# REEVALUATE/knowledge_enhanced_multimodal_retrieval

Measured on AMD Instinct MI355X. Metric: gallery images+texts encoded/sec (ViT-L/14; synthetic texts per SURVEY 8(d): end-of-text uniform in positions 8..76, mean 43.8 of 77 positions computed -- value_every_text_77_positions is the rate when every text fills the context) and 43k x Q sim+top-10 ms, higher is better.
Workload: dtype bf16; 1 GPU; CLIP ViT-L/14 zero-shot: 43k-gallery encode (1 image + query + target text per item, 224x224 / 77 tokens) + T2I top-10, BASELINE configs[1]; architecture=ViT-L/14, residual_stream=fp24, batch_per_gpu=255, text_group=1501, gallery=43000, parallelism=dp1 (gallery sharded), rccl_ranks=1

## Files before the change

knowledge_enhanced_multimodal_retrieval_amd/csrc/attention.hip:

```cpp
#include "common.h"

namespace kemr {

#ifndef KEMR_ATTN_PRIO
#define KEMR_ATTN_PRIO 0
#endif
__device__ __forceinline__ void attn_prio(int mfma_phase) {
    if constexpr (KEMR_ATTN_PRIO == 1) { if (mfma_phase) __builtin_amdgcn_s_setprio(1); else __builtin_amdgcn_s_setprio(0); }
    if constexpr (KEMR_ATTN_PRIO == 2) { if (mfma_phase) __builtin_amdgcn_s_setprio(0); else __builtin_amdgcn_s_setprio(1); }
}

template <bool NT>
__device__ __forceinline__ bf16x8 load_q8(const bf16_t* p) {
    if constexpr (NT) return __builtin_nontemporal_load((const bf16x8*)p);
    else return *(const bf16x8*)p;
}

template <int NT32, bool CAUSAL, int TC, int NW = 4, bool STAMP = false, int NTLOAD = 1, bool SKIPTAIL = false>
__global__ __launch_bounds__(NW * 64, 2) void attention_kernel(const bf16_t* __restrict__ qkv, bf16_t* __restrict__ out,
                                                           int T_rt, int width, int xbatch, const int* __restrict__ row_start) {
    constexpr int TP = NT32 * 32;
    constexpr int NT16 = NT32 * 2;
    constexpr int NTH = NW * 64;
    constexpr int NCH = (TP * 8 + NTH - 1) / NTH;
    constexpr float LOG2E = 1.4426950408889634f;
    extern __shared__ __attribute__((aligned(16))) char smem[];
    char* sK = smem;
    char* sV = smem + TP * 128;

    int h, b;
    if (!attn_item(xbatch, h, b)) return;
    int T_ = TC > 0 ? TC : T_rt;
    size_t row0 = (size_t)b * T_;
    if (TC == 0 && row_start) {
        const int r0 = row_start[b];
        T_ = row_start[b + 1] - r0;
        row0 = r0;
    }
    const int T = T_;
    const int tid = threadIdx.x, lane = tid & 63;
    const int wid = __builtin_amdgcn_readfirstlane(tid >> 6);
    const int ld = 3 * width;
    const bf16_t* base = qkv + row0 * ld + h * 64;
    const int lrow = lane & 15, lq = lane >> 4;
    const int nqt = SKIPTAIL ? T >> 4 : (T + 15) >> 4;

    unsigned long long st_t[8] = {0, 0, 0, 0, 0, 0, 0, 0}, st_prev = 0;
    auto stamp = [&](int k) {
        if constexpr (STAMP) {
            __builtin_amdgcn_sched_barrier(0);
            unsigned long long now;
            asm volatile("s_memtime %0\n\ts_waitcnt lgkmcnt(0)" : "=s"(now) :: "memory");
            __builtin_amdgcn_sched_barrier(0);
            st_t[k] += now - st_prev;
            st_prev = now;
        }
    };
    if constexpr (STAMP) { asm volatile("s_memtime %0\n\ts_waitcnt lgkmcnt(0)" : "=s"(st_prev) :: "memory"); __builtin_amdgcn_sched_barrier(0); }
    bf16x8 qn[2];
    {
        const int q0 = wid * 16 + lrow;
        const int qc = q0 < T ? q0 : T - 1;
#pragma unroll
        for (int kk = 0; kk < 2; ++kk) qn[kk] = load_q8<(NTLOAD >= 2)>(base + (size_t)qc * ld + kk * 32 + lq * 8);
    }
    {
        uint4 kv[NCH], vv[NCH];
#pragma unroll
        for (int i = 0; i < NCH; ++i) {
            const int idx = tid + i * NTH;
            const int row = idx >> 3, c = idx & 7;
            const int rc = row < T ? row : T - 1;
            if constexpr (NTLOAD >= 1) {
                typedef unsigned u32x4_ __attribute__((ext_vector_type(4)));
                const u32x4_ a_ = __builtin_nontemporal_load((const u32x4_*)(base + (size_t)rc * ld + width + c * 8));
                const u32x4_ b_ = __builtin_nontemporal_load((const u32x4_*)(base + (size_t)rc * ld + 2 * width + c * 8));
                kv[i] = make_uint4(a_.x, a_.y, a_.z, a_.w);
                vv[i] = make_uint4(b_.x, b_.y, b_.z, b_.w);
            } else {
                kv[i] = *(const uint4*)(base + (size_t)rc * ld + width + c * 8);
                vv[i] = *(const uint4*)(base + (size_t)rc * ld + 2 * width + c * 8);
            }
        }
#pragma unroll
        for (int i = 0; i < NCH; ++i) {
            const int idx = tid + i * NTH;
            const int row = idx >> 3, c = idx & 7;
            if (idx < TP * 8) {
                const unsigned keep = row < T ? 0xffffffffu : 0u;
                uint4 a = kv[i], b2 = vv[i];
                a.x &= keep; a.y &= keep; a.z &= keep; a.w &= keep;
                b2.x &= keep; b2.y &= keep; b2.z &= keep; b2.w &= keep;
                *(uint4*)(sK + row * 128 + ((c ^ ((row >> 1) & 7)) << 4)) = a;
                *(uint4*)(sV + row * 128 + ((c ^ (((row >> 1) & 3) << 1)) << 4)) = b2;
            }
        }
    }
    __syncthreads();
    stamp(0);

    for (int qt = wid; qt < nqt; qt += NW) {
        const int q = qt * 16 + lrow;
        bf16x8 qf[2] = {qn[0], qn[1]};
        if (qt + NW < nqt) {
            const int q2 = q + NW * 16;
            const int qc = q2 < T ? q2 : T - 1;
#pragma unroll
            for (int kk = 0; kk < 2; ++kk) qn[kk] = load_q8<(NTLOAD >= 2)>(base + (size_t)qc * ld + kk * 32 + lq * 8);
        }

        constexpr int G = (NT16 % 3 == 0) ? 3 : 2;
        constexpr int NG = NT16 / G;
        f32x4 s[NT16];
        bf16x8 kfr[2][G][2];
        auto load_group = [&](int g, bf16x8 (&dst)[G][2]) {
#pragma unroll
            for (int j = 0; j < G; ++j)
#pragma unroll
                for (int kk = 0; kk < 2; ++kk)
                    dst[j][kk] = *(const bf16x8*)(sK + ((g * G + j) * 16 + lrow) * 128 + (((kk * 4 + lq) ^ (lrow >> 1)) << 4));
        };
        load_group(0, kfr[0]);
        attn_prio(1);
#pragma unroll
        for (int g = 0; g < NG; ++g) {
            if (g + 1 < NG && (g + 1) * G * 16 < T) load_group(g + 1, kfr[(g + 1) & 1]);
            __builtin_amdgcn_sched_barrier(0);
#pragma unroll
            for (int j = 0; j < G; ++j) {
                const int t = g * G + j;
                s[t] = f32x4{0.f, 0.f, 0.f, 0.f};
                if (t * 16 < T && (!CAUSAL || t <= qt)) {
                    s[t] = __builtin_amdgcn_mfma_f32_16x16x32_bf16(kfr[g & 1][j][0], qf[0], s[t], 0, 0, 0);
                    s[t] = __builtin_amdgcn_mfma_f32_16x16x32_bf16(kfr[g & 1][j][1], qf[1], s[t], 0, 0, 0);
                }
            }
            __builtin_amdgcn_sched_barrier(0);
        }
        attn_prio(0);
        stamp(1);
        float mx = -INFINITY;
#pragma unroll
        for (int t = 0; t < NT16; ++t) {
            const bool partial = (t + 1) * 16 > T || CAUSAL;
#pragma unroll
            for (int r = 0; r < 4; ++r) {
                if (partial) {
                    const int key = t * 16 + lq * 4 + r;
                    const bool ok = key < T && (!CAUSAL || key <= q);
                    s[t][r] = ok ? s[t][r] : -INFINITY;
                }
                mx = fmaxf(mx, s[t][r]);
            }
        }
        mx = fmaxf(mx, __shfl_xor(mx, 16));
        mx = fmaxf(mx, __shfl_xor(mx, 32));
        const float mxl = mx * LOG2E;
        stamp(2);
        f32x2_t sum2 = {0.f, 0.f};
        const f32x2_t l2 = {LOG2E, LOG2E}, nm = {-mxl, -mxl};
        auto exp_tile = [&](int t) {
            f32x2_t a = f32x2_t{s[t][0], s[t][1]} * l2 + nm, c = f32x2_t{s[t][2], s[t][3]} * l2 + nm;
            a.x = __builtin_amdgcn_exp2f(a.x); a.y = __builtin_amdgcn_exp2f(a.y);
            c.x = __builtin_amdgcn_exp2f(c.x); c.y = __builtin_amdgcn_exp2f(c.y);
            s[t][0] = a.x; s[t][1] = a.y; s[t][2] = c.x; s[t][3] = c.y;
            sum2 += a;
            sum2 += c;
        };
#pragma unroll
        for (int t = 0; t < NT16; ++t) exp_tile(t);

        stamp(3);
        f32x4 o[4];
#pragma unroll
        for (int dt = 0; dt < 4; ++dt) o[dt] = f32x4{0.f, 0.f, 0.f, 0.f};
        bf16x8 vfr[2][4];
        auto load_v = [&](int u, bf16x8 (&dst)[4]) {
            const int ra = u * 32 + lq * 4 + (lrow >> 2);
            const int rb = ra + 16;
#pragma unroll
            for (int dt = 0; dt < 4; ++dt) {
                const int c = dt * 2 + ((lrow & 3) >> 1);
                const bf16x4 va = lds_read_tr16(sV + ra * 128 + ((c ^ (((ra >> 1) & 3) << 1)) << 4) + (lrow & 1) * 8);
                const bf16x4 vb = lds_read_tr16(sV + rb * 128 + ((c ^ (((rb >> 1) & 3) << 1)) << 4) + (lrow & 1) * 8);
                dst[dt][0] = va[0]; dst[dt][1] = va[1]; dst[dt][2] = va[2]; dst[dt][3] = va[3];
                dst[dt][4] = vb[0]; dst[dt][5] = vb[1]; dst[dt][6] = vb[2]; dst[dt][7] = vb[3];
            }
        };
        load_v(0, vfr[0]);
        attn_prio(1);
        auto live = [&](int u) { return u < NT32 && u * 32 < T && !(CAUSAL && u * 32 > qt * 16 + 15); };
#pragma unroll
        for (int u = 0; u < NT32; ++u) {
            if (!live(u)) continue;
            if (u + 1 < NT32 && (u + 1) * 32 < T) load_v(u + 1, vfr[(u + 1) & 1]);
            __builtin_amdgcn_sched_barrier(0);
            union { bf16x8 v; uint32_t w[4]; } pf;
            pf.w[0] = pack_bf16x2(s[2 * u][0], s[2 * u][1]);
            pf.w[1] = pack_bf16x2(s[2 * u][2], s[2 * u][3]);
            pf.w[2] = pack_bf16x2(s[2 * u + 1][0], s[2 * u + 1][1]);
            pf.w[3] = pack_bf16x2(s[2 * u + 1][2], s[2 * u + 1][3]);
#pragma unroll
            for (int dt = 0; dt < 4; ++dt)
                o[dt] = __builtin_amdgcn_mfma_f32_16x16x32_bf16(vfr[u & 1][dt], pf.v, o[dt], 0, 0, 0);
            __builtin_amdgcn_sched_barrier(0);
        }
        attn_prio(0);
        stamp(4);
        float sum = sum2.x + sum2.y;
        sum += __shfl_xor(sum, 16);
        sum += __shfl_xor(sum, 32);
        if (q < T) {
            const float inv = 1.0f / sum;
            bf16_t* dst = out + (row0 + q) * width + h * 64 + lq * 4;
#pragma unroll
            for (int dt = 0; dt < 4; ++dt) {
                uint2 pk;
                pk.x = pack_bf16x2(o[dt][0] * inv, o[dt][1] * inv);
                pk.y = pack_bf16x2(o[dt][2] * inv, o[dt][3] * inv);
                *(uint2*)(dst + dt * 16) = pk;
            }
        }
        stamp(5);
    }
    if constexpr (STAMP) {
        unsigned long long* dst = (unsigned long long*)(out + (size_t)xbatch * T * width) + (((size_t)b * (width >> 6) + h) * NW + wid) * 8;
        if (lane == 0) {
#pragma unroll
            for (int k = 0; k < 6; ++k) dst[k] += st_t[k];
            dst[6] += 1;
        }
    }
}

int g_attn_v = 0;

int g_attn_xcd = 1;
int g_attn_waves = 0;

#ifdef KEMR_AB_VARIANTS
int launch_attention_ab(int v, int waves, const bf16_t* qkv, bf16_t* out, int batch, int width, int xbatch, hipStream_t stream);
#endif

template <int NT32>
static int launch_nt(const bf16_t* qkv, bf16_t* out, int batch, int t, int width, int causal, hipStream_t stream, const int* row_start = nullptr) {
    constexpr int smem = NT32 * 32 * 128 * 2;
    const dim3 grid(width / 64, batch);
    ProfScope prof(PROF_ATTENTION, stream);
    void (*kern)(const bf16_t*, bf16_t*, int, int, int, const int*);
    const int xbatch = g_attn_xcd ? batch : 0;
    const dim3 xgrid(width / 64, xbatch ? (batch + 7) / 8 * 8 : batch);
    int threads = 256;
    if (causal) {
        if (NT32 == 3 && t == 77 && !row_start) { kern = attention_kernel<NT32, true, NT32 == 3 ? 77 : 0, NT32 == 3 ? 5 : 4>; threads = 320; }
        else kern = attention_kernel<NT32, true, 0>;
    } else if (NT32 == 9 && t == 257) {
#ifdef KEMR_AB_VARIANTS
        if (g_attn_v != 0) return launch_attention_ab(g_attn_v, g_attn_waves, qkv, out, batch, width, xbatch, stream);
        if (g_attn_waves == 6) { kern = attention_kernel<NT32, false, NT32 == 9 ? 257 : 0, NT32 == 9 ? 6 : 4>; threads = 384; }
        else if (g_attn_waves == 7) kern = attention_kernel<NT32, false, NT32 == 9 ? 257 : 0, 4, false, NT32 == 9 ? 0 : 1>;
        else if (g_attn_waves == 8) kern = attention_kernel<NT32, false, NT32 == 9 ? 257 : 0, 4, false, 1, NT32 == 9>;
        else if (g_attn_waves == 5) kern = attention_kernel<NT32, false, NT32 == 9 ? 257 : 0, 4, false, NT32 == 9 ? 2 : 1>;
        else if (g_attn_waves == 2 && xbatch) kern = attention_kernel<NT32, false, NT32 == 9 ? 257 : 0, 4, NT32 == 9>;
        else
#else
        if (g_attn_v != 0 || g_attn_waves != 0)
            KEMR_FAIL(KEMR_ERR_INVALID, "attention: attn_v = %d / attn_waves = %d select A/B kernels this library was built without (build.py --ab-variants)", g_attn_v, g_attn_waves);
#endif
        kern = attention_kernel<NT32, false, NT32 == 9 ? 257 : 0>;
    } else {
        kern = attention_kernel<NT32, false, 0>;
    }
    KEMR_CHECK_HIP(hipFuncSetAttribute((const void*)kern, hipFuncAttributeMaxDynamicSharedMemorySize, smem));
    hipLaunchKernelGGL(kern, xgrid, dim3(threads), smem, stream, qkv, out, t, width, xbatch, row_start);
    KEMR_CHECK_LAUNCH("attention_kernel");
    return KEMR_OK;
}

int launch_attention(const bf16_t* qkv, bf16_t* out, int batch, int t, int width, int causal, hipStream_t stream) {
    if (batch <= 0) return KEMR_OK;
    if (width % 64 != 0 || t <= 0) KEMR_FAIL(KEMR_ERR_INVALID, "attention: bad shape t=%d width=%d", t, width);
    if (batch > 65528) KEMR_FAIL(KEMR_ERR_INVALID, "attention: batch %d > 65528 (grid.y, rounded up to a multiple of 8)", batch);
    const int nt32 = (t + 31) / 32;
    switch (nt32) {
        case 1: return launch_nt<1>(qkv, out, batch, t, width, causal, stream);
        case 2: return launch_nt<2>(qkv, out, batch, t, width, causal, stream);
        case 3: return launch_nt<3>(qkv, out, batch, t, width, causal, stream);
        case 4: return launch_nt<4>(qkv, out, batch, t, width, causal, stream);
        case 5: return launch_nt<5>(qkv, out, batch, t, width, causal, stream);
        case 6: return launch_nt<6>(qkv, out, batch, t, width, causal, stream);
        case 7: return launch_nt<7>(qkv, out, batch, t, width, causal, stream);
        case 8: return launch_nt<8>(qkv, out, batch, t, width, causal, stream);
        case 9: return launch_nt<9>(qkv, out, batch, t, width, causal, stream);
    }
    if (!causal && t <= KEMR_MAX_VISION_TOKENS) return launch_attention_long(qkv, out, batch, t, width, stream);
    if (!causal) KEMR_FAIL(KEMR_ERR_INVALID, "attention: sequence length %d > %d not supported", t, KEMR_MAX_VISION_TOKENS);
    KEMR_FAIL(KEMR_ERR_INVALID, "attention: sequence length %d > 288 not supported (causal)", t);
}


template <int MAXK>
__global__ __launch_bounds__(256) void attention_pooled_kernel(const bf16_t* __restrict__ q, const bf16_t* __restrict__ qkv,
                                                               bf16_t* __restrict__ out, const int* __restrict__ pool_idx,
                                                               const int* __restrict__ row_start, int items, int tokens, int width,
                                                               int causal) {
    constexpr float LOG2E = 1.4426950408889634f;
    __shared__ float sp[4][MAXK];
    const int heads = width >> 6, lane = threadIdx.x & 63, wv = threadIdx.x >> 6;
    const int item = blockIdx.x * 4 + wv;
    if (item >= items * heads) return;
    const int b = item / heads, h = item - b * heads;
    const int r0 = row_start ? row_start[b] : b * tokens;
    int nk = causal ? pool_idx[b] - r0 + 1 : tokens;
    nk = nk < 1 ? 1 : (nk > MAXK ? MAXK : nk);
    const size_t ld = 3 * (size_t)width;
    const int ck = lane & 7, kq = lane >> 3;
    float qf[8];
    {
        const uint4 v = ((const uint4*)(q + (size_t)b * width + h * 64))[ck];
        const uint32_t w4[4] = {v.x, v.y, v.z, v.w};
#pragma unroll
        for (int k = 0; k < 4; ++k) {
            qf[2 * k] = bf16_to_f32((bf16_t)(w4[k] & 0xffff));
            qf[2 * k + 1] = bf16_to_f32((bf16_t)(w4[k] >> 16));
        }
    }
    const bf16_t* kbase = qkv + (size_t)r0 * ld + width + h * 64 + ck * 8;
    const int npass = (nk + 7) >> 3;
    for (int pss = 0; pss < npass; ++pss) {
        const int j = pss * 8 + kq;
        const int jc = j < nk ? j : nk - 1;
        const uint4 v = *(const uint4*)(kbase + (size_t)jc * ld);
        const uint32_t w4[4] = {v.x, v.y, v.z, v.w};
        float s = 0.f;
#pragma unroll
        for (int k = 0; k < 4; ++k) {
            s = fmaf(qf[2 * k], bf16_to_f32((bf16_t)(w4[k] & 0xffff)), s);
            s = fmaf(qf[2 * k + 1], bf16_to_f32((bf16_t)(w4[k] >> 16)), s);
        }
        s += __shfl_xor(s, 1);
        s += __shfl_xor(s, 2);
        s += __shfl_xor(s, 4);
        if (ck == 0 && j < nk) sp[wv][j] = s;
    }
    wave_lds_fence();
    float sc[MAXK / 64];
    float mx = -INFINITY;
#pragma unroll
    for (int pss = 0; pss < MAXK / 64; ++pss) {
        const int j = pss * 64 + lane;
        sc[pss] = j < nk ? sp[wv][j] : -INFINITY;
        mx = fmaxf(mx, sc[pss]);
    }
#pragma unroll
    for (int o = 32; o > 0; o >>= 1) mx = fmaxf(mx, __shfl_xor(mx, o));
    float sum = 0.f;
#pragma unroll
    for (int pss = 0; pss < MAXK / 64; ++pss) {
        const int j = pss * 64 + lane;
        const float p = __builtin_amdgcn_exp2f((sc[pss] - mx) * LOG2E);
        sum += p;
        if (j < MAXK) sp[wv][j] = bf16_to_f32(f32_to_bf16(p));
    }
#pragma unroll
    for (int o = 32; o > 0; o >>= 1) sum += __shfl_xor(sum, o);
    wave_lds_fence();
    const int dp = lane & 31, par = lane >> 5;
    const bf16_t* vp = qkv + (size_t)r0 * ld + 2 * width + h * 64 + dp * 2;
    float a0 = 0.f, a1 = 0.f;
#pragma unroll 4
    for (int j = par; j < nk; j += 2) {
        const uint32_t v = *(const uint32_t*)(vp + (size_t)j * ld);
        const float p = sp[wv][j];
        a0 = fmaf(p, bf16_to_f32((bf16_t)(v & 0xffff)), a0);
        a1 = fmaf(p, bf16_to_f32((bf16_t)(v >> 16)), a1);
    }
    a0 += __shfl_xor(a0, 32);
    a1 += __shfl_xor(a1, 32);
    if (par == 0) {
        const float inv = 1.0f / sum;
        *(uint32_t*)(out + (size_t)b * width + h * 64 + dp * 2) = pack_bf16x2(a0 * inv, a1 * inv);
    }
}

int launch_attention_pooled(const bf16_t* q, const bf16_t* qkv, bf16_t* out, const int* pool_idx, const int* row_start, int items,
                            int tokens, int width, int causal, hipStream_t stream, int force_long) {
    if (items <= 0) return KEMR_OK;
    if (width % 64 != 0 || tokens <= 0 || tokens > KEMR_MAX_VISION_TOKENS)
        KEMR_FAIL(KEMR_ERR_INVALID, "attention (pooled row): bad shape t=%d width=%d", tokens, width);
    if (causal && !pool_idx) KEMR_FAIL(KEMR_ERR_INVALID, "attention (pooled row): the causal form needs the pooled positions");
    ProfScope prof(PROF_ATTENTION, stream);
    const long waves = (long)items * (width / 64);
    constexpr int MAXK_LONG = (KEMR_MAX_VISION_TOKENS + 63) / 64 * 64;
    void (*kern)(const bf16_t*, const bf16_t*, bf16_t*, const int*, const int*, int, int, int, int) =
        tokens <= 320 && !force_long ? attention_pooled_kernel<320> : attention_pooled_kernel<MAXK_LONG>;
    hipLaunchKernelGGL(kern, dim3((unsigned)((waves + 3) / 4)), dim3(256), 0, stream, q, qkv, out, pool_idx, row_start, items, tokens,
                       width, causal);
    KEMR_CHECK_LAUNCH("attention_pooled_kernel");
    return KEMR_OK;
}

int launch_attention_packed(const bf16_t* qkv, bf16_t* out, const int* row_start, int batch, int max_t, int width, hipStream_t stream) {
    if (batch <= 0) return KEMR_OK;
    if (!row_start) KEMR_FAIL(KEMR_ERR_INVALID, "attention: packed rows need row_start");
    if (width % 64 != 0 || max_t <= 0) KEMR_FAIL(KEMR_ERR_INVALID, "attention: bad shape t=%d width=%d", max_t, width);
    if (batch > 65528) KEMR_FAIL(KEMR_ERR_INVALID, "attention: batch %d > 65528 (grid.y, rounded up to a multiple of 8)", batch);
    switch ((max_t + 31) / 32) {
        case 1: return launch_nt<1>(qkv, out, batch, max_t, width, 1, stream, row_start);
        case 2: return launch_nt<2>(qkv, out, batch, max_t, width, 1, stream, row_start);
        case 3: return launch_nt<3>(qkv, out, batch, max_t, width, 1, stream, row_start);
        case 4: return launch_nt<4>(qkv, out, batch, max_t, width, 1, stream, row_start);
    }
    return launch_attention_varlen_causal(qkv, out, row_start, batch, max_t, width, stream);
}

}
```

Baseline: 18700 items/s.

## Permute V columns in LDS so attention output stores are 16-byte wide

For compile-time sequence lengths (TC>0), V is written to LDS in 8-byte units under a new swizzle, so the PV MFMA output columns come out permuted. Each lane can then write its 16 contiguous output elements as two 16-byte stores instead of four 8-byte ones. The change also drops the row clamping and masking for load iterations that can never hit padding, and skips the max/exp work on key positions past TC that are known dead at compile time. In exchange the LDS write pattern changes (more, smaller stores, with possible bank conflicts) and the code gets more complicated.

```diff
diff --git a/knowledge_enhanced_multimodal_retrieval_amd/csrc/attention.hip b/knowledge_enhanced_multimodal_retrieval_amd/csrc/attention.hip
--- a/knowledge_enhanced_multimodal_retrieval_amd/csrc/attention.hip
+++ b/knowledge_enhanced_multimodal_retrieval_amd/csrc/attention.hip
@@ -4,6 +4,9 @@
 
 #ifndef KEMR_ATTN_PRIO
 #define KEMR_ATTN_PRIO 0
+#endif
+#ifndef KEMR_ATTN_WIDE_STORE
+#define KEMR_ATTN_WIDE_STORE 1
 #endif
 __device__ __forceinline__ void attn_prio(int mfma_phase) {
     if constexpr (KEMR_ATTN_PRIO == 1) { if (mfma_phase) __builtin_amdgcn_s_setprio(1); else __builtin_amdgcn_s_setprio(0); }
@@ -24,6 +27,7 @@
     constexpr int NTH = NW * 64;
     constexpr int NCH = (TP * 8 + NTH - 1) / NTH;
     constexpr float LOG2E = 1.4426950408889634f;
+    constexpr bool WIDE = TC > 0 && KEMR_ATTN_WIDE_STORE != 0;
     extern __shared__ __attribute__((aligned(16))) char smem[];
     char* sK = smem;
     char* sV = smem + TP * 128;
@@ -70,7 +74,8 @@
         for (int i = 0; i < NCH; ++i) {
             const int idx = tid + i * NTH;
             const int row = idx >> 3, c = idx & 7;
-            const int rc = row < T ? row : T - 1;
+            const bool pad_iter = TC == 0 || ((NTH - 1 + i * NTH) >> 3) >= TC;
+            const int rc = !pad_iter || row < T ? row : T - 1;
             if constexpr (NTLOAD >= 1) {
                 typedef unsigned u32x4_ __attribute__((ext_vector_type(4)));
                 const u32x4_ a_ = __builtin_nontemporal_load((const u32x4_*)(base + (size_t)rc * ld + width + c * 8));
@@ -87,12 +92,18 @@
             const int idx = tid + i * NTH;
             const int row = idx >> 3, c = idx & 7;
             if (idx < TP * 8) {
-                const unsigned keep = row < T ? 0xffffffffu : 0u;
+                const bool pad_iter = TC == 0 || ((NTH - 1 + i * NTH) >> 3) >= TC;
+                const unsigned keep = !pad_iter || row < T ? 0xffffffffu : 0u;
                 uint4 a = kv[i], b2 = vv[i];
                 a.x &= keep; a.y &= keep; a.z &= keep; a.w &= keep;
                 b2.x &= keep; b2.y &= keep; b2.z &= keep; b2.w &= keep;
                 *(uint4*)(sK + row * 128 + ((c ^ ((row >> 1) & 7)) << 4)) = a;
-                *(uint4*)(sV + row * 128 + ((c ^ (((row >> 1) & 3) << 1)) << 4)) = b2;
+                if constexpr (WIDE) {
+                    *(uint2*)(sV + row * 128 + (((2 * c) ^ ((row >> 1) & 3)) << 3)) = make_uint2(b2.x, b2.y);
+                    *(uint2*)(sV + row * 128 + (((2 * c + 1) ^ ((row >> 1) & 3)) << 3)) = make_uint2(b2.z, b2.w);
+                } else {
+                    *(uint4*)(sV + row * 128 + ((c ^ (((row >> 1) & 3) << 1)) << 4)) = b2;
+                }
             }
         }
     }
@@ -139,12 +150,14 @@
         }
         attn_prio(0);
         stamp(1);
+        auto dead = [](int t, int r) { return TC > 0 && t * 16 + r >= TC; };
         float mx = -INFINITY;
 #pragma unroll
         for (int t = 0; t < NT16; ++t) {
             const bool partial = (t + 1) * 16 > T || CAUSAL;
 #pragma unroll
             for (int r = 0; r < 4; ++r) {
+                if (dead(t, r)) continue;
                 if (partial) {
                     const int key = t * 16 + lq * 4 + r;
                     const bool ok = key < T && (!CAUSAL || key <= q);
@@ -160,6 +173,18 @@
         f32x2_t sum2 = {0.f, 0.f};
         const f32x2_t l2 = {LOG2E, LOG2E}, nm = {-mxl, -mxl};
         auto exp_tile = [&](int t) {
+            if (dead(t, 3)) {
+#pragma unroll
+                for (int r = 0; r < 4; ++r) {
+                    if (dead(t, r)) { s[t][r] = 0.f; continue; }
+                    float m = s[t][r] * LOG2E, nmx = -mxl;
+                    asm("" : "+v"(m), "+v"(nmx));
+                    const float e = __builtin_amdgcn_exp2f(m + nmx);
+                    s[t][r] = e;
+                    if (r & 1) sum2.y += e; else sum2.x += e;
+                }
+                return;
+            }
             f32x2_t a = f32x2_t{s[t][0], s[t][1]} * l2 + nm, c = f32x2_t{s[t][2], s[t][3]} * l2 + nm;
             a.x = __builtin_amdgcn_exp2f(a.x); a.y = __builtin_amdgcn_exp2f(a.y);
             c.x = __builtin_amdgcn_exp2f(c.x); c.y = __builtin_amdgcn_exp2f(c.y);
@@ -180,9 +205,16 @@
             const int rb = ra + 16;
 #pragma unroll
             for (int dt = 0; dt < 4; ++dt) {
-                const int c = dt * 2 + ((lrow & 3) >> 1);
-                const bf16x4 va = lds_read_tr16(sV + ra * 128 + ((c ^ (((ra >> 1) & 3) << 1)) << 4) + (lrow & 1) * 8);
-                const bf16x4 vb = lds_read_tr16(sV + rb * 128 + ((c ^ (((rb >> 1) & 3) << 1)) << 4) + (lrow & 1) * 8);
+                bf16x4 va, vb;
+                if constexpr (WIDE) {
+                    const int un = (lrow & 3) * 4 + dt;
+                    va = lds_read_tr16(sV + ra * 128 + ((un ^ ((ra >> 1) & 3)) << 3));
+                    vb = lds_read_tr16(sV + rb * 128 + ((un ^ ((rb >> 1) & 3)) << 3));
+                } else {
+                    const int c = dt * 2 + ((lrow & 3) >> 1);
+                    va = lds_read_tr16(sV + ra * 128 + ((c ^ (((ra >> 1) & 3) << 1)) << 4) + (lrow & 1) * 8);
+                    vb = lds_read_tr16(sV + rb * 128 + ((c ^ (((rb >> 1) & 3) << 1)) << 4) + (lrow & 1) * 8);
+                }
                 dst[dt][0] = va[0]; dst[dt][1] = va[1]; dst[dt][2] = va[2]; dst[dt][3] = va[3];
                 dst[dt][4] = vb[0]; dst[dt][5] = vb[1]; dst[dt][6] = vb[2]; dst[dt][7] = vb[3];
             }
@@ -212,13 +244,26 @@
         sum += __shfl_xor(sum, 32);
         if (q < T) {
             const float inv = 1.0f / sum;
-            bf16_t* dst = out + (row0 + q) * width + h * 64 + lq * 4;
-#pragma unroll
-            for (int dt = 0; dt < 4; ++dt) {
-                uint2 pk;
-                pk.x = pack_bf16x2(o[dt][0] * inv, o[dt][1] * inv);
-                pk.y = pack_bf16x2(o[dt][2] * inv, o[dt][3] * inv);
-                *(uint2*)(dst + dt * 16) = pk;
+            if constexpr (WIDE) {
+                bf16_t* dst = out + (row0 + q) * width + h * 64 + lq * 16;
+#pragma unroll
+                for (int half = 0; half < 2; ++half) {
+                    uint4 pk;
+                    pk.x = pack_bf16x2(o[2 * half][0] * inv, o[2 * half][1] * inv);
+                    pk.y = pack_bf16x2(o[2 * half][2] * inv, o[2 * half][3] * inv);
+                    pk.z = pack_bf16x2(o[2 * half + 1][0] * inv, o[2 * half + 1][1] * inv);
+                    pk.w = pack_bf16x2(o[2 * half + 1][2] * inv, o[2 * half + 1][3] * inv);
+                    *(uint4*)(dst + half * 8) = pk;
+                }
+            } else {
+                bf16_t* dst = out + (row0 + q) * width + h * 64 + lq * 4;
+#pragma unroll
+                for (int dt = 0; dt < 4; ++dt) {
+                    uint2 pk;
+                    pk.x = pack_bf16x2(o[dt][0] * inv, o[dt][1] * inv);
+                    pk.y = pack_bf16x2(o[dt][2] * inv, o[dt][3] * inv);
+                    *(uint2*)(dst + dt * 16) = pk;
+                }
             }
         }
         stamp(5);
```

Result: no change. 18760 items/s (median of 6 runs) (+0.3%).
